# oss0430/SRFRD

Hardware: AMD Instinct MI355X
Metric: sequences/sec (higher is better)
Workload: dtype f32

## Files before the change

include/srfrd_hip.h:

```cpp
#ifndef SRFRD_HIP_H
#define SRFRD_HIP_H

#include <stddef.h>
#include <stdint.h>

#ifdef __cplusplus
extern "C" {
#endif

#define SRFRD_MAX_BLOCKS 8
#define SRFRD_MAX_D 64

enum srfrd_kind {
  SRFRD_SASREC = 0,
  SRFRD_SRFR = 1,
  SRFRD_SRFRN = 2,
  SRFRD_SRFU_B = 3,
  SRFRD_SRFU_F = 4,
  SRFRD_SRFU_R = 5
};

enum srfrd_error {
  SRFRD_E_ARG = -1,
  SRFRD_E_UNSUPPORTED = -2,
// ... 128 lines not shown
int srfrd_reduce_dense(const float* grad_slabs, int n_slabs, int64_t n_dense, float* grad_dense,
                       const float* loss_part, int B, float* stats, float* loss_out, void* stream);

int srfrd_loss_stats(const float* loss_part, int B, float* stats, float* loss_out, void* stream);

int srfrd_step_begin(uint32_t* state, double lr, double beta1, double beta2, void* stream);

int srfrd_adam_step(float* param, float* grad, float* m, float* v, int64_t n, int64_t i0, int64_t i1,
                    int64_t n_zero, double beta1, double beta2, double eps,
                    const uint32_t* state, const float* stats, uint16_t* table_bf16, int64_t n_table, void* stream);

int srfrd_adam_pack_step(const srfrd_layout* lay, float* param, float* grad, float* m, float* v, int64_t n,
                         int64_t n_table_pad, int64_t n_zero, double lr, double beta1, double beta2, double eps,
                         uint32_t* state, const float* stats, float* packed, uint16_t* table_bf16, void* stream);

int srfrd_table_to_bf16(const float* src, int64_t n, uint16_t* out, void* stream);

int srfrd_l2_norms(const float* param, const int64_t* seg_off, const int64_t* seg_len, int n_seg, int64_t n_table_pad,
                   double l2_emb, float* partial, float* l2buf, float* dense_scale, void* stream);
int srfrd_l2_apply(float* grad, const float* param, int64_t i0, int64_t i1, int64_t n_table_pad, const float* l2buf,
                   const float* dense_scale, const float* stats, void* stream);

int srfrd_loss_finalize(const float* stats, float* loss_out, void* stream);

int srfrd_user_labels(int kind, const int64_t* fake_ids, int B, int L, int64_t* labels, void* stream);

int srfrd_check_ids(const int64_t* item_a, const int64_t* item_b, const int64_t* item_c,
                    const int64_t* fake_a, const int64_t* fake_b, const int64_t* fake_c,
                    int64_t n, int64_t n_items, int64_t fake_hi, uint32_t* err_word, void* stream);

// ... 75 lines not shown
```

srfrd_amd/_lib.py:

```python
from __future__ import annotations

import ctypes as C
import os

_HERE = os.path.dirname(os.path.abspath(__file__))
LIB_PATH = os.environ.get("SRFRD_LIB_PATH") or os.path.join(_HERE, "lib", "libsrfrd_hip.so")

MAX_BLOCKS = 8
MAX_D = 64
EXCL_CAP = 4096
KINDS = {"SASRec": 0, "SRFR": 1, "SRFRN": 2, "SRFU_B": 3, "SRFU_F": 4, "SRFU_R": 5}
_ERR = {-1: "SRFRD_E_ARG (bad argument)", -2: "SRFRD_E_UNSUPPORTED (configuration outside the fused kernels: "
        "hidden width > 64, hidden width not divisible by num_heads, a debug tap of a kernel without taps, or a caller-provided "
        "scratch buffer too small for this sequence length)", -3: "SRFRD_E_DEVICE"}


class BlockOff(C.Structure):
    _fields_ = [(n, C.c_int64) for n in ("ln1_w", "ln1_b", "in_w", "in_b", "out_w", "out_b", "ln2_w", "ln2_b",
                                         "c1_w", "c1_b", "c2_w", "c2_b")]


class Layout(C.Structure):
    _fields_ = ([(n, C.c_int32) for n in ("kind", "n_items", "max_len", "d_item", "d_fake", "D", "d_out", "n_labels",
                                          "n_blocks", "n_heads", "side_rows", "side_cols", "table_bf16", "reserved0")]
# ... 25 lines not shown
    "srfrd_encoder_fwd_sched": (_i, [_LP, _P, _P, _P, _P, _P, _P, _P, _P, _P, _i, _i, _d, _u32, _P, _i64,
                                     _P, _P, _P, _P, _P, _P, _P, _P, _i64, _P, _i, _P]),
    "srfrd_encoder_bwd_sched": (_i, [_LP, _P, _P, _P, _P, _P, _P, _P, _P, _P, _i, _i, _d, _u32, _P, _i64,
                                     _P, _P, _P, _P, _P, _P, _P, _P, _P, _i, _P, _P, _P, _P, _i64, _P, _i, _P]),
    "srfrd_encoder_plan_train": (_i, [_LP, _i, _i, _i, _i, _i, _i64, _P, _i, _P]),
    "srfrd_train_scratch_floats": (_i64, [_LP, _i, _i]),
    "srfrd_encoder_train_sched": (_i, [_LP, _P, _P, _P, _P, _P, _P, _P, _P, _P, _i, _i, _d, _u32, _P, _i64,
                                       _P, _P, _P, _P, _P, _P, _P, _P, _P, _P, _i, _P, _P, _P, _P, _i64, _P, _i, _P]),
    "srfrd_table_reduce": (_i, [_P, _P, _P, _i64, _i, _P, _P]),
    "srfrd_aux_floats": (_i64, [_LP, _i, _i]),
    "srfrd_reduce_dense": (_i, [_P, _i, _i64, _P, _P, _i, _P, _P, _P]),
    "srfrd_loss_stats": (_i, [_P, _i, _P, _P, _P]),
    "srfrd_step_begin": (_i, [_P, _d, _d, _d, _P]),
    "srfrd_adam_step": (_i, [_P, _P, _P, _P, _i64, _i64, _i64, _i64, _d, _d, _d, _P, _P, _P, _i64, _P]),
    "srfrd_adam_pack_step": (_i, [_LP, _P, _P, _P, _P, _i64, _i64, _i64, _d, _d, _d, _d, _P, _P, _P, _P, _P]),
    "srfrd_table_to_bf16": (_i, [_P, _i64, _P, _P]),
    "srfrd_loss_finalize": (_i, [_P, _P, _P]),
    "srfrd_l2_norms": (_i, [_P, _P, _P, _i, _i64, _d, _P, _P, _P, _P]),
    "srfrd_l2_apply": (_i, [_P, _P, _i64, _i64, _i64, _P, _P, _P, _P]),
    "srfrd_user_labels": (_i, [_i, _P, _i, _i, _P, _P]),
    "srfrd_check_ids": (_i, [_P, _P, _P, _P, _P, _P, _i64, _i64, _i64, _P, _P]),
    "srfrd_predict_logits": (_i, [_LP, _P, _P, _P, _i, _i, _P, _i, _i64, _P, _P, _P]),
    "srfrd_topk_workspace_bytes": (_i64, [_i, _i, _i64]),
    "srfrd_logits_topk": (_i, [_LP, _P, _P, _P, _i, _i, _i64, _i64, _i, _P, _i, _P, _P, _P, _P]),
    "srfrd_topk_merge": (_i, [_P, _P, _i, _i, _i, _P, _P, _P]),
    "srfrd_excl_workspace_bytes": (_i64, [_i, _i, _i64]),
    "srfrd_logits_topk_excl": (_i, [_LP, _P, _P, _P, _i, _i, _i64, _i64, _i, _P, _i, _P, _P, _i, _P, _P, _P, _P, _P]),
    "srfrd_target_rank": (_i, [_LP, _P, _P, _P, _i, _i, _i64, _i64, _i, _P, _P, _P, _P, _i, _i, _P, _P, _P, _P]),
    "srfrd_rank_plan": (_i, [_LP, _i, _i, _i, _i64, _i64, _i, _i, _i, _i, _P, _i, _P]),
    "srfrd_eval_rank": (_i, [_P, _i, _i, _P, _P, _P]),
# ... 105 lines not shown
```

srfrd_amd/csrc/srfrd_optim.hip:

```cpp
#include "srfrd_dev.h"

namespace srfrd {

__global__ void __launch_bounds__(256) reduce_dense_kernel(const float* __restrict__ slabs, int n_slabs, int64_t n_dense,
                                                          float* __restrict__ grad_dense, const float* __restrict__ loss_part,
                                                          int B, float* __restrict__ stats, float* __restrict__ loss_out) {
  __shared__ float part[4][64];
  const int lane = threadIdx.x & 63, wave = threadIdx.x >> 6;
  const int64_t i = (int64_t)blockIdx.x * 64 + lane;
  float s0 = 0.f, s1 = 0.f, s2 = 0.f, s3 = 0.f;
  if (i < n_dense) {
    int w = wave;
    for (; w + 28 < n_slabs; w += 32) {
      const float a0 = slabs[(int64_t)w * n_dense + i], a1 = slabs[(int64_t)(w + 4) * n_dense + i];
      const float a2 = slabs[(int64_t)(w + 8) * n_dense + i], a3 = slabs[(int64_t)(w + 12) * n_dense + i];
      const float a4 = slabs[(int64_t)(w + 16) * n_dense + i], a5 = slabs[(int64_t)(w + 20) * n_dense + i];
      const float a6 = slabs[(int64_t)(w + 24) * n_dense + i], a7 = slabs[(int64_t)(w + 28) * n_dense + i];
      s0 += a0; s1 += a1; s2 += a2; s3 += a3;
      s0 += a4; s1 += a5; s2 += a6; s3 += a7;
    }
    for (; w + 12 < n_slabs; w += 16) {
      s0 += slabs[(int64_t)w * n_dense + i];
      s1 += slabs[(int64_t)(w + 4) * n_dense + i];
      s2 += slabs[(int64_t)(w + 8) * n_dense + i];
      s3 += slabs[(int64_t)(w + 12) * n_dense + i];
    }
    for (; w < n_slabs; w += 4) s0 += slabs[(int64_t)w * n_dense + i];
  }
  part[wave][lane] = (s0 + s1) + (s2 + s3);
  __syncthreads();
  if (wave == 0 && i < n_dense) grad_dense[i] = (part[0][lane] + part[1][lane]) + (part[2][lane] + part[3][lane]);
  if (blockIdx.x == 0 && loss_part != nullptr && stats != nullptr) {
    __shared__ float red[4][3];
    float a0 = 0.f, a1 = 0.f, a2 = 0.f;
    for (int b = threadIdx.x; b < B; b += blockDim.x) {
      a0 += loss_part[(int64_t)b * 3 + 0];
      a1 += loss_part[(int64_t)b * 3 + 1];
      a2 += loss_part[(int64_t)b * 3 + 2];
    }
    a0 = wave_sum(a0); a1 = wave_sum(a1); a2 = wave_sum(a2);
    if (lane == 0) { red[wave][0] = a0; red[wave][1] = a1; red[wave][2] = a2; }
    __syncthreads();
    if (threadIdx.x < 3) {
      float s = 0.f;
      for (int w = 0; w < 4; ++w) s += red[w][threadIdx.x];
      stats[threadIdx.x] = s;
      red[0][threadIdx.x] = s;
    }
    if (threadIdx.x == 3) stats[3] = 0.f;
    if (loss_out != nullptr) {
      __syncthreads();
      if (threadIdx.x == 0) loss_out[0] = red[0][0] / red[0][2] + red[0][1] / red[0][2];
    }
  }
}

__global__ void __launch_bounds__(256) loss_stats_kernel(const float* __restrict__ loss_part, int B, float* __restrict__ stats,
                                                        float* __restrict__ loss_out) {
  __shared__ float red[4][3];
  const int lane = threadIdx.x & 63, wave = threadIdx.x >> 6;
  float a0 = 0.f, a1 = 0.f, a2 = 0.f;
  for (int b = threadIdx.x; b < B; b += blockDim.x) {
    a0 += loss_part[(int64_t)b * 3 + 0];
    a1 += loss_part[(int64_t)b * 3 + 1];
    a2 += loss_part[(int64_t)b * 3 + 2];
  }
  a0 = wave_sum(a0); a1 = wave_sum(a1); a2 = wave_sum(a2);
  if (lane == 0) { red[wave][0] = a0; red[wave][1] = a1; red[wave][2] = a2; }
// ... 21 lines not shown
  for (int64_t j = i; j < n && keys[j] == key; ++j)
    if (lane < di) acc += contrib[order[j] * di + lane];
  if (lane < di) grad_table[key * di + lane] = acc;
}

__global__ void step_begin_kernel(uint32_t* state, double lr, double b1, double b2) {
  if (threadIdx.x == 0 && blockIdx.x == 0) step_advance(state, lr, b1, b2);
}

__device__ __forceinline__ void adam_one(float& p, float g, float& m, float& v, float b1, float b2, float eps,
                                         float step_size, float bc2s) {
  m = m * b1 + (1.0f - b1) * g;
  v = v * b2 + ((1.0f - b2) * g) * g;
  const float denom = sqrtf(v) / bc2s + eps;
  p = p - step_size * (m / denom);
}

__device__ __forceinline__ void shadow_store4(uint16_t* __restrict__ shadow, int64_t i, int64_t n_shadow, const float4& p4) {
  const uint16_t h0 = f32_to_bf16(p4.x), h1 = f32_to_bf16(p4.y), h2 = f32_to_bf16(p4.z), h3 = f32_to_bf16(p4.w);
  if (i + 3 < n_shadow) {
    *reinterpret_cast<uint2*>(shadow + i) = make_uint2((uint32_t)h0 | ((uint32_t)h1 << 16), (uint32_t)h2 | ((uint32_t)h3 << 16));
  } else {
    shadow[i] = h0;
    if (i + 1 < n_shadow) shadow[i + 1] = h1;
    if (i + 2 < n_shadow) shadow[i + 2] = h2;
  }
}

__global__ void __launch_bounds__(256) table_to_bf16_kernel(const float* __restrict__ src, int64_t n, uint16_t* __restrict__ out) {
  const int64_t stride = (int64_t)gridDim.x * blockDim.x;
// ... 55 lines not shown
    else if (off >= o.c2_w && off < o.c2_w + DD) { m = 5; e = off - o.c2_w; }
    else return;
    mat = b * 6 + m; N = D; K = D;
  }
  (void)N;
  const int n = e / K, k = e - n * K;
  auto slot = [](int kk, int nn) {
    const int rem = kk & 15;
    return ((nn >> 4) << 10) | ((kk >> 4) << 8) | ((((rem & 3) << 4) | (nn & 15)) << 2) | (rem >> 2);
  };
  float* base = packed + (int64_t)mat * 2 * kPackFloats;
  base[slot(k, n)] = val;
  base[kPackFloats + slot(n, k)] = val;
}

__global__ void __launch_bounds__(512) adam_pack_kernel(float* __restrict__ param, float* __restrict__ grad, float* __restrict__ m,
                                                       float* __restrict__ v, int64_t n, int64_t n_tab, int64_t n_zero, float b1,
                                                       float b2, float eps, uint32_t* __restrict__ state,
                                                       const float* __restrict__ stats, Dims dims, float* __restrict__ packed,
                                                       double lr, double b1d, double b2d, uint16_t* __restrict__ shadow,
                                                       int64_t n_shadow) {
  const float step_size = ((const float*)state)[4];
  const float bc2s = ((const float*)state)[5];
  const float gscale = stats ? 1.0f / stats[2] : 1.0f;
  const int64_t nvec = n >> 2;
  const int64_t stride = (int64_t)gridDim.x * blockDim.x;
  const int64_t w_lo = n_tab + dims.blk0;
  for (int64_t q = (int64_t)blockIdx.x * blockDim.x + threadIdx.x; q < nvec; q += stride) {
    const int64_t i = q << 2;
    float4 p4 = *reinterpret_cast<float4*>(param + i);
    float4 g4 = *reinterpret_cast<const float4*>(grad + i);
    float4 m4 = *reinterpret_cast<float4*>(m + i);
    float4 v4 = *reinterpret_cast<float4*>(v + i);
    adam_one(p4.x, g4.x * gscale, m4.x, v4.x, b1, b2, eps, step_size, bc2s);
    adam_one(p4.y, g4.y * gscale, m4.y, v4.y, b1, b2, eps, step_size, bc2s);
    adam_one(p4.z, g4.z * gscale, m4.z, v4.z, b1, b2, eps, step_size, bc2s);
    adam_one(p4.w, g4.w * gscale, m4.w, v4.w, b1, b2, eps, step_size, bc2s);
    *reinterpret_cast<float4*>(param + i) = p4;
    *reinterpret_cast<float4*>(m + i) = m4;
    *reinterpret_cast<float4*>(v + i) = v4;
    if (i + 3 < n_zero) *reinterpret_cast<float4*>(grad + i) = make_float4(0.f, 0.f, 0.f, 0.f);
    else if (i < n_zero) for (int k = 0; k < 4; ++k) if (i + k < n_zero) grad[i + k] = 0.f;
    if (shadow != nullptr && i < n_shadow) shadow_store4(shadow, i, n_shadow, p4);
    if (i + 3 >= w_lo) {
      pack_scatter(dims, i - n_tab, p4.x, packed);
      pack_scatter(dims, i + 1 - n_tab, p4.y, packed);
      pack_scatter(dims, i + 2 - n_tab, p4.z, packed);
      pack_scatter(dims, i + 3 - n_tab, p4.w, packed);
    }
  }
  for (int64_t i = (nvec << 2) + (int64_t)blockIdx.x * blockDim.x + threadIdx.x; i < n; i += stride) {
    float p = param[i], mm = m[i], vv = v[i];
    adam_one(p, grad[i] * gscale, mm, vv, b1, b2, eps, step_size, bc2s);
    param[i] = p; m[i] = mm; v[i] = vv;
    if (i < n_zero) grad[i] = 0.f;
    if (shadow != nullptr && i < n_shadow) shadow[i] = f32_to_bf16(p);
    if (i >= w_lo) pack_scatter(dims, i - n_tab, p, packed);
  }
  __syncthreads();
  if (threadIdx.x == 0) {
    const unsigned shard = blockIdx.x & 15u, n_shards = gridDim.x < 16u ? gridDim.x : 16u;
    const unsigned in_shard = (gridDim.x - shard + 15u) >> 4;
    if (atomicAdd(&state[8 + shard], 1u) == in_shard - 1u) {
      state[8 + shard] = 0;
      if (atomicAdd(&state[6], 1u) == n_shards - 1u) {
        state[6] = 0;
        step_advance(state, lr, b1d, b2d);
      }
    }
  }
}

__global__ void __launch_bounds__(256) l2_partial_kernel(const float* __restrict__ param, const int64_t* __restrict__ seg_off,
                                                        const int64_t* __restrict__ seg_len, int n_tw, float* __restrict__ partial) {
  __shared__ float red[4];
  const int g = blockIdx.x;
  int64_t lo, hi;
  if (g < n_tw) {
    const int64_t n = seg_len[0], per = ((n + n_tw - 1) / n_tw + 3) & ~3ll;
    lo = seg_off[0] + g * per;
    hi = seg_off[0] + (g + 1) * per < seg_off[0] + n ? seg_off[0] + (g + 1) * per : seg_off[0] + n;
  } else {
    const int k = g - n_tw + 1;
    lo = seg_off[k];
    hi = lo + seg_len[k];
// ... 100 lines not shown

extern "C" int srfrd_adam_step(float* param, float* grad, float* m, float* v, int64_t n, int64_t i0, int64_t i1,
                               int64_t n_zero, double beta1, double beta2, double eps, const uint32_t* state,
                               const float* stats, uint16_t* table_bf16, int64_t n_table, void* stream) {
  if (!param || !grad || !m || !v || !state || n <= 0 || i0 < 0 || i1 > n || i0 > i1) return SRFRD_E_ARG;
  if (i0 == i1) return 0;
  if (i0 & 3) return SRFRD_E_ARG;
  const int64_t nvec = ((i1 - i0) >> 2) + 1;
  int64_t grid = (nvec + 255) / 256;
  if (grid > 4096) grid = 4096;
  hipLaunchKernelGGL(adam_kernel, dim3((int)grid), dim3(256), 0, (hipStream_t)stream, param, grad, m, v, i0, i1, n_zero,
                     (float)beta1, (float)beta2, (float)eps, state, stats, table_bf16, table_bf16 ? n_table : 0);
  return (int)hipGetLastError();
}

extern "C" int srfrd_adam_pack_step(const srfrd_layout* lay, float* param, float* grad, float* m, float* v, int64_t n,
                                    int64_t n_table_pad, int64_t n_zero, double lr, double beta1, double beta2, double eps,
                                    uint32_t* state, const float* stats, float* packed, uint16_t* table_bf16, void* stream) {
  if (!lay || !param || !grad || !m || !v || !state || !packed || n <= 0 || n_table_pad < 0 || (n_table_pad & 3) ||
      n_table_pad + lay->n_dense > n)
    return SRFRD_E_ARG;
  if (lay->D > SRFRD_MAX_D) return SRFRD_E_UNSUPPORTED;
  Dims d = {};
  d.kind = lay->kind; d.d_item = lay->d_item; d.d_fake = lay->d_fake; d.D = lay->D; d.d_out = lay->d_out;
  d.n_labels = lay->n_labels; d.n_blocks = lay->n_blocks;
  d.off_pos = (int)lay->off_pos; d.off_side = (int)lay->off_side;
  d.blk0 = lay->n_blocks > 0 ? (int)lay->blk[0].ln1_w : 0;
  d.blk_stride = blk_stride_of(lay->D);
  d.off_lc_w = (int)lay->off_lc_w; d.off_lc_b = (int)lay->off_lc_b; d.off_ll_w = (int)lay->off_ll_w; d.off_ll_b = (int)lay->off_ll_b;
  d.n_dense = (int)lay->n_dense;
  int64_t grid = ((n >> 2) + 1 + 511) / 512;
  if (grid > 768) grid = 768;
  hipLaunchKernelGGL(adam_pack_kernel, dim3((int)grid), dim3(512), 0, (hipStream_t)stream, param, grad, m, v, n, n_table_pad,
                     n_zero, (float)beta1, (float)beta2, (float)eps, state, stats, d, packed, lr, beta1, beta2, table_bf16,
                     table_bf16 ? lay->n_table : 0);
  return (int)hipGetLastError();
}

extern "C" int srfrd_l2_norms(const float* param, const int64_t* seg_off, const int64_t* seg_len, int n_seg, int64_t n_table_pad,
                              double l2_emb, float* partial, float* l2buf, float* dense_scale, void* stream) {
  if (!param || !seg_off || !seg_len || !partial || !l2buf || !dense_scale || n_seg < 1 || n_seg > 128 || n_table_pad < 0)
    return SRFRD_E_ARG;
  const int n_tw = 240;
  hipLaunchKernelGGL(l2_partial_kernel, dim3(n_tw + n_seg - 1), dim3(256), 0, (hipStream_t)stream, param, seg_off, seg_len, n_tw,
                     partial);
  hipLaunchKernelGGL(l2_finish_kernel, dim3(1), dim3(256), 0, (hipStream_t)stream, partial, seg_off, seg_len, n_seg, n_tw,
                     n_table_pad, (float)l2_emb, l2buf, dense_scale);
  return (int)hipGetLastError();
}

// ... 17 lines not shown
```

srfrd_amd/trainer.py:

```python
from __future__ import annotations

import ctypes as C
import os

import torch
import torch.distributed as dist

import numpy as np

from . import _lib, loss_heads
from ._lib import check, ptr
from .exchange import GradExchange, exchange_active, shard_bounds
from .sampler import alias_table, negative_q

LOSSES = ("bce", "sampled_softmax", "softmax")


def flat_allreduce(flat: torch.Tensor, group=None):
    if dist.is_available() and dist.is_initialized() and dist.get_world_size(group) > 1:
        dist.all_reduce(flat, op=dist.ReduceOp.SUM, group=group)
    return flat


def _loss_config(model, loss, num_negatives, neg_counts, neg_alpha, process_group):
# ... 168 lines not shown

    def _dense_ptr(self, base):
        return C.c_void_p(base.data_ptr() + 4 * self.n_tab)

    def _ids_of(self, slot):
        ids = self.ids_ring[slot]
        fk = ids[1] if self.lay.kind != 0 else None
        pfk, nfk = (ids[3], ids[5]) if self.lay.kind == 2 else (None, None)
        p = self.model.dropout_rate if self.model.training else 0.0
        return ids, fk, pfk, nfk, p, C.c_void_p(self.state.data_ptr() + 8), self.rank * self.B

    def _enqueue_l2_apply(self, grad_ptr, param, i0, i1):
        check(_lib.lib().srfrd_l2_apply(grad_ptr, ptr(param), i0, min(i1, self.n_flat), self.n_tab, ptr(self.l2buf),
                                        ptr(self.l2_dense), ptr(self.stats), self._stream()), "srfrd_l2_apply")

    def _enqueue_fwd(self, slot: int = 0, train: bool = False):
        L_, lay, st = _lib.lib(), self.lay, self._stream()
        if self.l2 != 0.0:
            check(L_.srfrd_l2_norms(ptr(self.flat), ptr(self.seg_off), ptr(self.seg_len), self.seg_off.numel(), self.n_tab,
                                    self.l2, ptr(self.l2_partial), ptr(self.l2buf), ptr(self.l2_dense), st), "srfrd_l2_norms")
        ids, fk, pfk, nfk, p, seed_dev, seq0 = self._ids_of(slot)
        lay_t, tab = self.model._table_args()
        if self.sched_mode:
            check(L_.srfrd_seq_order(ptr(ids[0]), self.B, self.L, self.pair_stride, ptr(self.sched), st), "srfrd_seq_order")
        if train:
            check(L_.srfrd_encoder_train_sched(C.byref(lay_t), tab, self._dense_ptr(self.flat), ptr(self.packed), ptr(ids[0]), ptr(fk),
                                               ptr(ids[2]), ptr(pfk), ptr(ids[4]), ptr(nfk), self.B, self.L, p, 0, seed_dev, seq0,
                                               ptr(self.hidden), ptr(self.pl), ptr(self.nl), ptr(self.save_x), ptr(self.save_h1),
                                               ptr(self.save_aux), ptr(self.loss_part), None, None, None, 1, ptr(self.grad),
                                               ptr(self.contrib), ptr(self.slabs), ptr(self.scratch), self.n_scratch, ptr(self.sched),
                                               self.sched_mode, st), "srfrd_encoder_train_sched")
            self._enqueue_grad_tail(slot)
            return
        check(L_.srfrd_encoder_fwd_sched(C.byref(lay_t), tab, self._dense_ptr(self.flat), ptr(self.packed), ptr(ids[0]), ptr(fk), ptr(ids[2]),
                                         ptr(pfk), ptr(ids[4]), ptr(nfk), self.B, self.L, p, 0, seed_dev, seq0, ptr(self.hidden),
                                         ptr(self.pl), ptr(self.nl), ptr(self.save_x), ptr(self.save_h1), ptr(self.save_aux), ptr(self.loss_part),
                                         ptr(self.scratch), self.n_scratch, ptr(self.sched), self.sched_mode, st), "srfrd_encoder_fwd_sched")
        if self.mode == "sharded":
            check(L_.srfrd_loss_stats(ptr(self.loss_part), self.B, ptr(self.stats), None, st), "srfrd_loss_stats")

    def _enqueue_bwd(self, slot: int = 0):
        L_, lay, st = _lib.lib(), self.lay, self._stream()
        ids, fk, pfk, nfk, p, seed_dev, seq0 = self._ids_of(slot)
        lay_t, tab = self.model._table_args()
        check(L_.srfrd_encoder_bwd_sched(C.byref(lay_t), tab, self._dense_ptr(self.flat), ptr(self.packed), ptr(ids[0]), ptr(fk), ptr(ids[2]),
                                         ptr(pfk), ptr(ids[4]), ptr(nfk), self.B, self.L, p, 0, seed_dev, seq0, ptr(self.hidden),
                                         ptr(self.pl), ptr(self.nl), ptr(self.save_x), ptr(self.save_h1), ptr(self.save_aux), None, None, None, 1,
                                         ptr(self.grad), ptr(self.contrib), ptr(self.slabs), ptr(self.scratch), self.n_scratch,
                                         ptr(self.sched), self.sched_mode, st), "srfrd_encoder_bwd_sched")
        self._enqueue_grad_tail(slot)

    def _enqueue_grad_tail(self, slot: int = 0):
        L_, lay, st = _lib.lib(), self.lay, self._stream()
        ids = self.ids_ring[slot]
        if self.contrib is not None:
            torch.stack((ids[2], ids[4], ids[0]), out=self.keys)
            skeys, order = torch.sort(self.keys.view(-1), stable=True)
            check(L_.srfrd_table_reduce(ptr(skeys), ptr(order), ptr(self.contrib), skeys.numel(), lay.d_item, ptr(self.grad), st),
                  "srfrd_table_reduce")
        fuse_stats = self.mode != "sharded"
        check(L_.srfrd_reduce_dense(ptr(self.slabs), self.n_slabs, lay.n_dense, self._dense_ptr(self.grad),
                                    ptr(self.loss_part) if fuse_stats else None, self.B, ptr(self.stats) if fuse_stats else None,
                                    ptr(self.loss) if self.mode == "single" else None, st), "srfrd_reduce_dense")

    def _enqueue_ce_compute(self, slot: int = 0):
        L_, lay, st = _lib.lib(), self.lay, self._stream()
        B, L, T, di = self.B, self.L, self.B * self.L, lay.d_item
        if self.l2 != 0.0:
            check(L_.srfrd_l2_norms(ptr(self.flat), ptr(self.seg_off), ptr(self.seg_len), self.seg_off.numel(), self.n_tab,
                                    self.l2, ptr(self.l2_partial), ptr(self.l2buf), ptr(self.l2_dense), st), "srfrd_l2_norms")
        ids, fk, pfk, nfk, p, seed_dev, seq0 = self._ids_of(slot)
        lay_t, tab = self.model._table_args()
        if self.sched_mode:
            check(L_.srfrd_seq_order(ptr(ids[0]), B, L, self.pair_stride, ptr(self.sched), st), "srfrd_seq_order")
# ... 39 lines not shown
              "srfrd_reduce_dense")

    def _enqueue_compute(self, slot: int = 0):
        self._enqueue_fwd(slot)
        self._enqueue_bwd(slot)

    def _enqueue_step_compute(self, slot: int = 0):
        if self.loss_kind != "bce":
            self._enqueue_ce_compute(slot)
        elif self.mode == "single" and self.train_launch and _lib.encoder_plan_train(
                self.lay, self.B, self.L, self._train_mode, _lib.env_switches())[0]:
            self._enqueue_fwd(slot, train=True)
        else:
            self._enqueue_compute(slot)

    def _enqueue_update(self):
        L_, st = _lib.lib(), self._stream()
        if self.l2 != 0.0:
            self._enqueue_l2_apply(ptr(self.grad), self.flat, 0, self.n_flat)
        check(L_.srfrd_adam_pack_step(C.byref(self.lay), ptr(self.flat), ptr(self.grad), ptr(self.m), ptr(self.v),
                                      self.n_flat, self.n_tab, self.n_tab, self.lr, self.betas[0], self.betas[1], self.eps,
                                      ptr(self.state), ptr(self.stats), ptr(self.packed), ptr(self.model._table16), st),
              "srfrd_adam_pack_step")
        if self.mode != "single" or self.loss_kind != "bce":
            check(L_.srfrd_loss_finalize(ptr(self.stats), ptr(self.loss), st), "srfrd_loss_finalize")
        if self.l2 != 0.0:
            self.loss.add_(self.l2buf[1:2])

    def _enqueue_shard_update(self):
        L_, st, ex = _lib.lib(), self._stream(), self.ex
# ... 48 lines not shown
                h.wait()
            self._enqueue_shard_update()
            self._gather_params()
            self._enqueue_shard_finish()

    def _capture(self):
        torch.cuda.synchronize()
        keep = [self.flat, self.m, self.v, self.state, self.grad, self.stats] + ([self.shadow_pad] if self.shadow_gather else [])
        snap = [t.clone() for t in keep]
        s = torch.cuda.Stream()
        s.wait_stream(torch.cuda.current_stream())
        with torch.cuda.stream(s):
            if self.mode != "single" and self.ex.native:
                self._enqueue_dp_step()
            else:
                self._enqueue_step_compute()
                if self.mode == "sharded":
                    self._enqueue_shard_update()
                    self._enqueue_shard_finish()
                else:
                    self._enqueue_update()
        torch.cuda.current_stream().wait_stream(s)
        torch.cuda.synchronize()

        def restore():
            for dst, src in zip(keep, snap):
                dst.copy_(src)
            self.model.pack_weights()
            if not self.shadow_gather:
                self.model.refresh_bf16_table()

        restore()

        def graph_of(fn):
            g = torch.cuda.CUDAGraph()
            with torch.cuda.graph(g, capture_error_mode="thread_local"):
# ... 1 lines not shown
            return g

        self.graph_form = "one" if self.mode == "single" else "split"
        if self.mode != "single" and self.ex.native and os.environ.get("SRFRD_DP_SPLIT_GRAPHS", "") != "1":
            try:
                self._graph_one = [graph_of(lambda k=k: self._enqueue_dp_step(k)) for k in range(self.slots)]
                self.graph_form = "one"
            except Exception as e:
                self._graph_one = None
                self.graph_capture_error = repr(e)
                torch.cuda.synchronize()
                restore()
        if self.graph_form == "one" and self.mode != "single":
            pass
        elif self.mode == "single":
            self._graph_a = [graph_of(lambda k=k: (self._enqueue_step_compute(k), self._enqueue_update())) for k in range(self.slots)]
        elif self.mode == "allreduce":
            self._graph_a = [graph_of(lambda k=k: self._enqueue_compute(k)) for k in range(self.slots)]
            self._graph_b = graph_of(self._enqueue_update)
        else:
            self._graph_f = [graph_of(lambda k=k: self._enqueue_fwd(k)) for k in range(self.slots)]
            self._graph_a = [graph_of(lambda k=k: self._enqueue_bwd(k)) for k in range(self.slots)]
            self._graph_u = graph_of(self._enqueue_shard_update)
            self._graph_b = graph_of(self._enqueue_shard_finish)
        if self._graph_one is None:
            for gs in (self._graph_f, self._graph_a, [self._graph_u], [self._graph_b]):
                for g in (gs or []):
                    if g is not None:
                        g.replay()
        else:
            for g in self._graph_one:
# ... 136 lines not shown
        return self._run()

    def step_slot(self, slot: int) -> torch.Tensor:
        if not 0 <= slot < self.slots:
            raise IndexError(f"slot {slot} outside the ring of {self.slots}")
        return self._run(slot)

    def _run(self, slot: int = 0):
        if not self._fresh:
            self.refresh()
        g = self.use_graph
        if g and self._graph_a is None and self._graph_one is None:
            self._capture()
        if not g:
            if self.mode == "single":
                self._enqueue_step_compute(slot)
                self._enqueue_update()
            else:
                self._enqueue_dp_step(slot)
        elif self._graph_one is not None:
            self._graph_one[slot].replay()
        elif self.mode == "single":
            self._graph_a[slot].replay()
        elif self.mode == "allreduce":
            self._graph_a[slot].replay()
            self.ex.all_reduce(self.grad)
            self._graph_b.replay()
        else:
            self._graph_f[slot].replay()
            h = self.ex.all_reduce_stats(self.stats)
            self._graph_a[slot].replay()
            self.ex.reduce_scatter(self.grad, self.recv)
# ... 8 lines not shown
```

Baseline: 3.050 million.

## Fuse dense slab reduction, loss stats and Adam pack step into one kernel

```diff
diff --git a/include/srfrd_hip.h b/include/srfrd_hip.h
--- a/include/srfrd_hip.h
+++ b/include/srfrd_hip.h
@@ -166,6 +166,11 @@
                          int64_t n_table_pad, int64_t n_zero, double lr, double beta1, double beta2, double eps,
                          uint32_t* state, const float* stats, float* packed, uint16_t* table_bf16, void* stream);
 
+int srfrd_reduce_adam_pack_step(const srfrd_layout* lay, const float* grad_slabs, int n_slabs, const float* loss_part, int B,
+                                int L, float* stats, float* loss_out, float* param, float* grad, float* m, float* v, int64_t n,
+                                int64_t n_table_pad, int64_t n_zero, double lr, double beta1, double beta2, double eps,
+                                uint32_t* state, float* packed, uint16_t* table_bf16, void* stream);
+
 int srfrd_table_to_bf16(const float* src, int64_t n, uint16_t* out, void* stream);
 
 int srfrd_l2_norms(const float* param, const int64_t* seg_off, const int64_t* seg_len, int n_seg, int64_t n_table_pad,
diff --git a/srfrd_amd/_lib.py b/srfrd_amd/_lib.py
--- a/srfrd_amd/_lib.py
+++ b/srfrd_amd/_lib.py
@@ -63,6 +63,8 @@
     "srfrd_step_begin": (_i, [_P, _d, _d, _d, _P]),
     "srfrd_adam_step": (_i, [_P, _P, _P, _P, _i64, _i64, _i64, _i64, _d, _d, _d, _P, _P, _P, _i64, _P]),
     "srfrd_adam_pack_step": (_i, [_LP, _P, _P, _P, _P, _i64, _i64, _i64, _d, _d, _d, _d, _P, _P, _P, _P, _P]),
+    "srfrd_reduce_adam_pack_step": (_i, [_LP, _P, _i, _P, _i, _i, _P, _P, _P, _P, _P, _P, _i64, _i64, _i64, _d, _d, _d, _d,
+                                         _P, _P, _P, _P]),
     "srfrd_table_to_bf16": (_i, [_P, _i64, _P, _P]),
     "srfrd_loss_finalize": (_i, [_P, _P, _P]),
     "srfrd_l2_norms": (_i, [_P, _P, _P, _i, _i64, _d, _P, _P, _P, _P]),
diff --git a/srfrd_amd/csrc/srfrd_optim.hip b/srfrd_amd/csrc/srfrd_optim.hip
--- a/srfrd_amd/csrc/srfrd_optim.hip
+++ b/srfrd_amd/csrc/srfrd_optim.hip
@@ -1,6 +1,65 @@
 #include "srfrd_dev.h"
 
 namespace srfrd {
+
+template <bool DEEP = false>
+__device__ __forceinline__ float slab_quarter_sum(const float* __restrict__ slabs, int n_slabs, int64_t n_dense, int64_t i, int w) {
+  float s0 = 0.f, s1 = 0.f, s2 = 0.f, s3 = 0.f;
+  if constexpr (DEEP) {
+    for (; w + 60 < n_slabs; w += 64) {
+      float a[16];
+#pragma unroll
+      for (int k = 0; k < 16; ++k) a[k] = slabs[(int64_t)(w + 4 * k) * n_dense + i];
+      s0 += a[0]; s1 += a[1]; s2 += a[2]; s3 += a[3];
+      s0 += a[4]; s1 += a[5]; s2 += a[6]; s3 += a[7];
+      s0 += a[8]; s1 += a[9]; s2 += a[10]; s3 += a[11];
+      s0 += a[12]; s1 += a[13]; s2 += a[14]; s3 += a[15];
+    }
+  }
+  for (; w + 28 < n_slabs; w += 32) {
+    const float a0 = slabs[(int64_t)w * n_dense + i], a1 = slabs[(int64_t)(w + 4) * n_dense + i];
+    const float a2 = slabs[(int64_t)(w + 8) * n_dense + i], a3 = slabs[(int64_t)(w + 12) * n_dense + i];
+    const float a4 = slabs[(int64_t)(w + 16) * n_dense + i], a5 = slabs[(int64_t)(w + 20) * n_dense + i];
+    const float a6 = slabs[(int64_t)(w + 24) * n_dense + i], a7 = slabs[(int64_t)(w + 28) * n_dense + i];
+    s0 += a0; s1 += a1; s2 += a2; s3 += a3;
+    s0 += a4; s1 += a5; s2 += a6; s3 += a7;
+  }
+  for (; w + 12 < n_slabs; w += 16) {
+    s0 += slabs[(int64_t)w * n_dense + i];
+    s1 += slabs[(int64_t)(w + 4) * n_dense + i];
+    s2 += slabs[(int64_t)(w + 8) * n_dense + i];
+    s3 += slabs[(int64_t)(w + 12) * n_dense + i];
+  }
+  for (; w < n_slabs; w += 4) s0 += slabs[(int64_t)w * n_dense + i];
+  return (s0 + s1) + (s2 + s3);
+}
+
+__device__ __forceinline__ void loss_tree(const float* __restrict__ loss_part, int B, float* __restrict__ stats,
+                                          float* __restrict__ loss_out, float (*red)[3]) {
+  const int lane = threadIdx.x & 63, wave = threadIdx.x >> 6;
+  float a0 = 0.f, a1 = 0.f, a2 = 0.f;
+  if (threadIdx.x < 256) {
+    for (int b = threadIdx.x; b < B; b += 256) {
+      a0 += loss_part[(int64_t)b * 3 + 0];
+      a1 += loss_part[(int64_t)b * 3 + 1];
+      a2 += loss_part[(int64_t)b * 3 + 2];
+    }
+  }
+  a0 = wave_sum(a0); a1 = wave_sum(a1); a2 = wave_sum(a2);
+  if (lane == 0 && wave < 4) { red[wave][0] = a0; red[wave][1] = a1; red[wave][2] = a2; }
+  __syncthreads();
+  if (threadIdx.x < 3) {
+    float s = 0.f;
+    for (int w = 0; w < 4; ++w) s += red[w][threadIdx.x];
+    stats[threadIdx.x] = s;
+    red[0][threadIdx.x] = s;
+  }
+  if (threadIdx.x == 3) stats[3] = 0.f;
+  if (loss_out != nullptr) {
+    __syncthreads();
+    if (threadIdx.x == 0) loss_out[0] = red[0][0] / red[0][2] + red[0][1] / red[0][2];
+  }
+}
 
 __global__ void __launch_bounds__(256) reduce_dense_kernel(const float* __restrict__ slabs, int n_slabs, int64_t n_dense,
                                                           float* __restrict__ grad_dense, const float* __restrict__ loss_part,
@@ -8,50 +67,12 @@
   __shared__ float part[4][64];
   const int lane = threadIdx.x & 63, wave = threadIdx.x >> 6;
   const int64_t i = (int64_t)blockIdx.x * 64 + lane;
-  float s0 = 0.f, s1 = 0.f, s2 = 0.f, s3 = 0.f;
-  if (i < n_dense) {
-    int w = wave;
-    for (; w + 28 < n_slabs; w += 32) {
-      const float a0 = slabs[(int64_t)w * n_dense + i], a1 = slabs[(int64_t)(w + 4) * n_dense + i];
-      const float a2 = slabs[(int64_t)(w + 8) * n_dense + i], a3 = slabs[(int64_t)(w + 12) * n_dense + i];
-      const float a4 = slabs[(int64_t)(w + 16) * n_dense + i], a5 = slabs[(int64_t)(w + 20) * n_dense + i];
-      const float a6 = slabs[(int64_t)(w + 24) * n_dense + i], a7 = slabs[(int64_t)(w + 28) * n_dense + i];
-      s0 += a0; s1 += a1; s2 += a2; s3 += a3;
-      s0 += a4; s1 += a5; s2 += a6; s3 += a7;
-    }
-    for (; w + 12 < n_slabs; w += 16) {
-      s0 += slabs[(int64_t)w * n_dense + i];
-      s1 += slabs[(int64_t)(w + 4) * n_dense + i];
-      s2 += slabs[(int64_t)(w + 8) * n_dense + i];
-      s3 += slabs[(int64_t)(w + 12) * n_dense + i];
-    }
-    for (; w < n_slabs; w += 4) s0 += slabs[(int64_t)w * n_dense + i];
-  }
-  part[wave][lane] = (s0 + s1) + (s2 + s3);
+  part[wave][lane] = i < n_dense ? slab_quarter_sum(slabs, n_slabs, n_dense, i, wave) : 0.f;
   __syncthreads();
   if (wave == 0 && i < n_dense) grad_dense[i] = (part[0][lane] + part[1][lane]) + (part[2][lane] + part[3][lane]);
   if (blockIdx.x == 0 && loss_part != nullptr && stats != nullptr) {
     __shared__ float red[4][3];
-    float a0 = 0.f, a1 = 0.f, a2 = 0.f;
-    for (int b = threadIdx.x; b < B; b += blockDim.x) {
-      a0 += loss_part[(int64_t)b * 3 + 0];
-      a1 += loss_part[(int64_t)b * 3 + 1];
-      a2 += loss_part[(int64_t)b * 3 + 2];
-    }
-    a0 = wave_sum(a0); a1 = wave_sum(a1); a2 = wave_sum(a2);
-    if (lane == 0) { red[wave][0] = a0; red[wave][1] = a1; red[wave][2] = a2; }
-    __syncthreads();
-    if (threadIdx.x < 3) {
-      float s = 0.f;
-      for (int w = 0; w < 4; ++w) s += red[w][threadIdx.x];
-      stats[threadIdx.x] = s;
-      red[0][threadIdx.x] = s;
-    }
-    if (threadIdx.x == 3) stats[3] = 0.f;
-    if (loss_out != nullptr) {
-      __syncthreads();
-      if (threadIdx.x == 0) loss_out[0] = red[0][0] / red[0][2] + red[0][1] / red[0][2];
-    }
+    loss_tree(loss_part, B, stats, loss_out, red);
   }
 }
 
@@ -103,6 +124,14 @@
   v = v * b2 + ((1.0f - b2) * g) * g;
   const float denom = sqrtf(v) / bc2s + eps;
   p = p - step_size * (m / denom);
+}
+
+__device__ __forceinline__ void adam_one_pinned(float& p, float g, float& m, float& v, float b1, float b2, float eps,
+                                                float step_size, float bc2s) {
+  m = __fmaf_rn(1.0f - b1, g, __fmul_rn(m, b1));
+  v = __fmaf_rn(g, __fmul_rn(1.0f - b2, g), __fmul_rn(v, b2));
+  const float denom = __fadd_rn(sqrtf(v) / bc2s, eps);
+  p = __fmaf_rn(-step_size, m / denom, p);
 }
 
 __device__ __forceinline__ void shadow_store4(uint16_t* __restrict__ shadow, int64_t i, int64_t n_shadow, const float4& p4) {
@@ -188,6 +217,56 @@
   base[kPackFloats + slot(n, k)] = val;
 }
 
+template <bool PIN>
+__device__ __forceinline__ float4 adam_vec4_step(float* __restrict__ param, float* __restrict__ grad, float* __restrict__ m,
+                                                 float* __restrict__ v, int64_t i, int64_t n_zero, float b1, float b2, float eps,
+                                                 float step_size, float bc2s, float gscale, uint16_t* __restrict__ shadow,
+                                                 int64_t n_shadow, float4 p4, float4 g4, float4 m4, float4 v4) {
+  if constexpr (PIN) {
+    adam_one_pinned(p4.x, g4.x * gscale, m4.x, v4.x, b1, b2, eps, step_size, bc2s);
+    adam_one_pinned(p4.y, g4.y * gscale, m4.y, v4.y, b1, b2, eps, step_size, bc2s);
+    adam_one_pinned(p4.z, g4.z * gscale, m4.z, v4.z, b1, b2, eps, step_size, bc2s);
+    adam_one_pinned(p4.w, g4.w * gscale, m4.w, v4.w, b1, b2, eps, step_size, bc2s);
+  } else {
+    adam_one(p4.x, g4.x * gscale, m4.x, v4.x, b1, b2, eps, step_size, bc2s);
+    adam_one(p4.y, g4.y * gscale, m4.y, v4.y, b1, b2, eps, step_size, bc2s);
+    adam_one(p4.z, g4.z * gscale, m4.z, v4.z, b1, b2, eps, step_size, bc2s);
+    adam_one(p4.w, g4.w * gscale, m4.w, v4.w, b1, b2, eps, step_size, bc2s);
+  }
+  *reinterpret_cast<float4*>(param + i) = p4;
+  *reinterpret_cast<float4*>(m + i) = m4;
+  *reinterpret_cast<float4*>(v + i) = v4;
+  if (i + 3 < n_zero) *reinterpret_cast<float4*>(grad + i) = make_float4(0.f, 0.f, 0.f, 0.f);
+  else if (i < n_zero) for (int k = 0; k < 4; ++k) if (i + k < n_zero) grad[i + k] = 0.f;
+  if (shadow != nullptr && i < n_shadow) shadow_store4(shadow, i, n_shadow, p4);
+  return p4;
+}
+template <bool PIN>
+__device__ __forceinline__ float4 adam_vec4(float* __restrict__ param, float* __restrict__ grad, float* __restrict__ m,
+                                            float* __restrict__ v, int64_t i, int64_t n_zero, float b1, float b2, float eps,
+                                            float step_size, float bc2s, float gscale, uint16_t* __restrict__ shadow, int64_t n_shadow) {
+  const float4 p4 = *reinterpret_cast<float4*>(param + i);
+  const float4 g4 = *reinterpret_cast<const float4*>(grad + i);
+  const float4 m4 = *reinterpret_cast<float4*>(m + i);
+  const float4 v4 = *reinterpret_cast<float4*>(v + i);
+  return adam_vec4_step<PIN>(param, grad, m, v, i, n_zero, b1, b2, eps, step_size, bc2s, gscale, shadow, n_shadow, p4, g4, m4, v4);
+}
+
+__device__ __forceinline__ void step_ticket(uint32_t* __restrict__ state, double lr, double b1d, double b2d) {
+  __syncthreads();
+  if (threadIdx.x == 0) {
+    const unsigned shard = blockIdx.x & 15u, n_shards = gridDim.x < 16u ? gridDim.x : 16u;
+    const unsigned in_shard = (gridDim.x - shard + 15u) >> 4;
+    if (atomicAdd(&state[8 + shard], 1u) == in_shard - 1u) {
+      state[8 + shard] = 0;
+      if (atomicAdd(&state[6], 1u) == n_shards - 1u) {
+        state[6] = 0;
+        step_advance(state, lr, b1d, b2d);
+      }
+    }
+  }
+}
+
 __global__ void __launch_bounds__(512) adam_pack_kernel(float* __restrict__ param, float* __restrict__ grad, float* __restrict__ m,
                                                        float* __restrict__ v, int64_t n, int64_t n_tab, int64_t n_zero, float b1,
                                                        float b2, float eps, uint32_t* __restrict__ state,
@@ -202,20 +281,7 @@
   const int64_t w_lo = n_tab + dims.blk0;
   for (int64_t q = (int64_t)blockIdx.x * blockDim.x + threadIdx.x; q < nvec; q += stride) {
     const int64_t i = q << 2;
-    float4 p4 = *reinterpret_cast<float4*>(param + i);
-    float4 g4 = *reinterpret_cast<const float4*>(grad + i);
-    float4 m4 = *reinterpret_cast<float4*>(m + i);
-    float4 v4 = *reinterpret_cast<float4*>(v + i);
-    adam_one(p4.x, g4.x * gscale, m4.x, v4.x, b1, b2, eps, step_size, bc2s);
-    adam_one(p4.y, g4.y * gscale, m4.y, v4.y, b1, b2, eps, step_size, bc2s);
-    adam_one(p4.z, g4.z * gscale, m4.z, v4.z, b1, b2, eps, step_size, bc2s);
-    adam_one(p4.w, g4.w * gscale, m4.w, v4.w, b1, b2, eps, step_size, bc2s);
-    *reinterpret_cast<float4*>(param + i) = p4;
-    *reinterpret_cast<float4*>(m + i) = m4;
-    *reinterpret_cast<float4*>(v + i) = v4;
-    if (i + 3 < n_zero) *reinterpret_cast<float4*>(grad + i) = make_float4(0.f, 0.f, 0.f, 0.f);
-    else if (i < n_zero) for (int k = 0; k < 4; ++k) if (i + k < n_zero) grad[i + k] = 0.f;
-    if (shadow != nullptr && i < n_shadow) shadow_store4(shadow, i, n_shadow, p4);
+    const float4 p4 = adam_vec4<false>(param, grad, m, v, i, n_zero, b1, b2, eps, step_size, bc2s, gscale, shadow, n_shadow);
     if (i + 3 >= w_lo) {
       pack_scatter(dims, i - n_tab, p4.x, packed);
       pack_scatter(dims, i + 1 - n_tab, p4.y, packed);
@@ -231,18 +297,98 @@
     if (shadow != nullptr && i < n_shadow) shadow[i] = f32_to_bf16(p);
     if (i >= w_lo) pack_scatter(dims, i - n_tab, p, packed);
   }
-  __syncthreads();
-  if (threadIdx.x == 0) {
-    const unsigned shard = blockIdx.x & 15u, n_shards = gridDim.x < 16u ? gridDim.x : 16u;
-    const unsigned in_shard = (gridDim.x - shard + 15u) >> 4;
-    if (atomicAdd(&state[8 + shard], 1u) == in_shard - 1u) {
-      state[8 + shard] = 0;
-      if (atomicAdd(&state[6], 1u) == n_shards - 1u) {
-        state[6] = 0;
-        step_advance(state, lr, b1d, b2d);
+  step_ticket(state, lr, b1d, b2d);
+}
+
+__global__ void __launch_bounds__(512) reduce_adam_pack_kernel(const float* __restrict__ slabs, int n_slabs, int64_t n_dense,
+                                                              const float* __restrict__ loss_part, int B, float* __restrict__ stats,
+                                                              float* __restrict__ loss_out, float* __restrict__ param,
+                                                              float* __restrict__ grad, float* __restrict__ m, float* __restrict__ v,
+                                                              int64_t n, int64_t n_tab, int64_t n_zero, float b1, float b2, float eps,
+                                                              uint32_t* __restrict__ state, Dims dims, float* __restrict__ packed,
+                                                              double lr, double b1d, double b2d, uint16_t* __restrict__ shadow,
+                                                              int64_t n_shadow, int dense_first, int n_dense_blocks) {
+  __shared__ float part[2][4][64];
+  __shared__ float red[4][3];
+  __shared__ float cred[8];
+  const int tid = threadIdx.x, lane = tid & 63, wave = tid >> 6;
+  const float step_size = ((const float*)state)[4];
+  const float bc2s = ((const float*)state)[5];
+  const int bid = blockIdx.x;
+  const bool dense_role = bid >= dense_first && bid < dense_first + n_dense_blocks;
+  const bool table_role = !dense_role || gridDim.x == 1;
+  float cnt = 0.f;
+  for (int b = tid; b < B; b += 512) cnt += loss_part[(int64_t)b * 3 + 2];
+  if (bid == 0) loss_tree(loss_part, B, stats, loss_out, red);
+  const int half = wave >> 2, w4 = wave & 3;
+  const int64_t n_pairs = (((n_dense + 63) >> 6) + 1) >> 1;
+  const int64_t u0 = bid - dense_first;
+  float mine = 0.f, p0 = 0.f, m0 = 0.f, v0 = 0.f;
+  if (dense_role && u0 < n_pairs) {
+    const int64_t j = ((u0 << 1) + half) * 64 + lane;
+    if (j < n_dense) {
+      if (w4 == 0) { p0 = param[n_tab + j]; m0 = m[n_tab + j]; v0 = v[n_tab + j]; }
+      mine = slab_quarter_sum<true>(slabs, n_slabs, n_dense, j, w4);
+    }
+  }
+  const int64_t nvec = n_tab >> 2;
+  const int64_t t_blocks = (int64_t)gridDim.x - (gridDim.x == 1 ? 0 : n_dense_blocks);
+  const int64_t t_index = bid == 0 ? 0 : bid - n_dense_blocks;
+  const int64_t stride = t_blocks * 512;
+  int64_t q = t_index * 512 + tid;
+  float4 p4, g4, m4, v4;
+  const bool first = table_role && bid != 0 && q < nvec;
+  if (first) {
+    p4 = *reinterpret_cast<const float4*>(param + (q << 2));
+    g4 = *reinterpret_cast<const float4*>(grad + (q << 2));
+    m4 = *reinterpret_cast<const float4*>(m + (q << 2));
+    v4 = *reinterpret_cast<const float4*>(v + (q << 2));
+  }
+  cnt = wave_sum(cnt);
+  if (lane == 0) cred[wave] = cnt;
+  part[half][w4][lane] = mine;
+  __syncthreads();
+  float count = 0.f;
+  for (int w = 0; w < 8; ++w) count += cred[w];
+  const float gscale = 1.0f / count;
+  const int64_t w_lo = n_tab + dims.blk0;
+  if (dense_role) {
+    for (int64_t u = u0; u < n_pairs; u += n_dense_blocks) {
+      const int64_t j = ((u << 1) + half) * 64 + lane;
+      if (u != u0) {
+        part[half][w4][lane] = j < n_dense ? slab_quarter_sum<true>(slabs, n_slabs, n_dense, j, w4) : 0.f;
+        __syncthreads();
       }
-    }
-  }
+      if (w4 == 0 && j < n_dense) {
+        const float gd = (part[half][0][lane] + part[half][1][lane]) + (part[half][2][lane] + part[half][3][lane]);
+        const int64_t i = n_tab + j;
+        grad[i] = gd;
+        float p = p0, mm = m0, vv = v0;
+        if (u != u0) { p = param[i]; mm = m[i]; vv = v[i]; }
+        adam_one_pinned(p, gd * gscale, mm, vv, b1, b2, eps, step_size, bc2s);
+        param[i] = p; m[i] = mm; v[i] = vv;
+        if (i >= w_lo) pack_scatter(dims, j, p, packed);
+      }
+      __syncthreads();
+    }
+  }
+  if (bid == 0) {
+    for (int64_t i = n_tab + n_dense + tid; i < n; i += 512) {
+      float p = param[i], mm = m[i], vv = v[i];
+      adam_one_pinned(p, grad[i] * gscale, mm, vv, b1, b2, eps, step_size, bc2s);
+      param[i] = p; m[i] = mm; v[i] = vv;
+      if (i >= w_lo) pack_scatter(dims, i - n_tab, p, packed);
+    }
+  }
+  if (table_role) {
+    if (first) {
+      adam_vec4_step<true>(param, grad, m, v, q << 2, n_zero, b1, b2, eps, step_size, bc2s, gscale, shadow, n_shadow, p4, g4, m4, v4);
+      q += stride;
+    }
+    for (; q < nvec; q += stride)
+      adam_vec4<true>(param, grad, m, v, q << 2, n_zero, b1, b2, eps, step_size, bc2s, gscale, shadow, n_shadow);
+  }
+  step_ticket(state, lr, b1d, b2d);
 }
 
 __global__ void __launch_bounds__(256) l2_partial_kernel(const float* __restrict__ param, const int64_t* __restrict__ seg_off,
@@ -373,13 +519,7 @@
   return (int)hipGetLastError();
 }
 
-extern "C" int srfrd_adam_pack_step(const srfrd_layout* lay, float* param, float* grad, float* m, float* v, int64_t n,
-                                    int64_t n_table_pad, int64_t n_zero, double lr, double beta1, double beta2, double eps,
-                                    uint32_t* state, const float* stats, float* packed, uint16_t* table_bf16, void* stream) {
-  if (!lay || !param || !grad || !m || !v || !state || !packed || n <= 0 || n_table_pad < 0 || (n_table_pad & 3) ||
-      n_table_pad + lay->n_dense > n)
-    return SRFRD_E_ARG;
-  if (lay->D > SRFRD_MAX_D) return SRFRD_E_UNSUPPORTED;
+static Dims optim_dims(const srfrd_layout* lay) {
   Dims d = {};
   d.kind = lay->kind; d.d_item = lay->d_item; d.d_fake = lay->d_fake; d.D = lay->D; d.d_out = lay->d_out;
   d.n_labels = lay->n_labels; d.n_blocks = lay->n_blocks;
@@ -388,11 +528,49 @@
   d.blk_stride = blk_stride_of(lay->D);
   d.off_lc_w = (int)lay->off_lc_w; d.off_lc_b = (int)lay->off_lc_b; d.off_ll_w = (int)lay->off_ll_w; d.off_ll_b = (int)lay->off_ll_b;
   d.n_dense = (int)lay->n_dense;
+  return d;
+}
+
+extern "C" int srfrd_adam_pack_step(const srfrd_layout* lay, float* param, float* grad, float* m, float* v, int64_t n,
+                                    int64_t n_table_pad, int64_t n_zero, double lr, double beta1, double beta2, double eps,
+                                    uint32_t* state, const float* stats, float* packed, uint16_t* table_bf16, void* stream) {
+  if (!lay || !param || !grad || !m || !v || !state || !packed || n <= 0 || n_table_pad < 0 || (n_table_pad & 3) ||
+      n_table_pad + lay->n_dense > n)
+    return SRFRD_E_ARG;
+  if (lay->D > SRFRD_MAX_D) return SRFRD_E_UNSUPPORTED;
+  const Dims d = optim_dims(lay);
   int64_t grid = ((n >> 2) + 1 + 511) / 512;
   if (grid > 768) grid = 768;
   hipLaunchKernelGGL(adam_pack_kernel, dim3((int)grid), dim3(512), 0, (hipStream_t)stream, param, grad, m, v, n, n_table_pad,
                      n_zero, (float)beta1, (float)beta2, (float)eps, state, stats, d, packed, lr, beta1, beta2, table_bf16,
                      table_bf16 ? lay->n_table : 0);
+  return (int)hipGetLastError();
+}
+
+extern "C" int srfrd_reduce_adam_pack_step(const srfrd_layout* lay, const float* grad_slabs, int n_slabs, const float* loss_part,
+                                           int B, int L, float* stats, float* loss_out, float* param, float* grad, float* m,
+                                           float* v, int64_t n, int64_t n_table_pad, int64_t n_zero, double lr, double beta1,
+                                           double beta2, double eps, uint32_t* state, float* packed, uint16_t* table_bf16,
+                                           void* stream) {
+  if (!lay || !grad_slabs || !loss_part || !stats || !loss_out || !param || !grad || !m || !v || !state || !packed) return SRFRD_E_ARG;
+  if (n_slabs <= 0 || B <= 0 || L <= 0 || lay->n_dense <= 0 || n <= 0 || n_table_pad < 0 || (n_table_pad & 3) ||
+      n_table_pad + lay->n_dense > n || n_zero < 0 || n_zero > n_table_pad || lay->n_table > n_table_pad)
+    return SRFRD_E_ARG;
+  if (lay->D > SRFRD_MAX_D) return SRFRD_E_UNSUPPORTED;
+  if ((int64_t)B * L >= (1ll << 24)) return SRFRD_E_UNSUPPORTED;
+  const Dims d = optim_dims(lay);
+  int64_t grid = ((n >> 2) + 1 + 511) / 512;
+  if (grid > 768) grid = 768;
+  const int64_t n_pairs = (((lay->n_dense + 63) >> 6) + 1) >> 1;
+  const double dense_bytes = 4.0 * n_slabs * (double)lay->n_dense, table_bytes = 32.0 * (double)n_table_pad;
+  int64_t nd = (int64_t)((double)grid * dense_bytes / (dense_bytes + table_bytes) + 0.5);
+  if (nd > n_pairs) nd = n_pairs;
+  if (nd > grid - 1) nd = grid - 1;
+  if (nd < 1) nd = 1;
+  hipLaunchKernelGGL(reduce_adam_pack_kernel, dim3((int)grid), dim3(512), 0, (hipStream_t)stream, grad_slabs, n_slabs,
+                     (int64_t)lay->n_dense, loss_part, B, stats, loss_out, param, grad, m, v, n, n_table_pad, n_zero, (float)beta1,
+                     (float)beta2, (float)eps, state, d, packed, lr, beta1, beta2, table_bf16, table_bf16 ? lay->n_table : 0,
+                     grid > 1 ? 1 : 0, (int)nd);
   return (int)hipGetLastError();
 }
 
diff --git a/srfrd_amd/trainer.py b/srfrd_amd/trainer.py
--- a/srfrd_amd/trainer.py
+++ b/srfrd_amd/trainer.py
@@ -206,7 +206,7 @@
         check(_lib.lib().srfrd_l2_apply(grad_ptr, ptr(param), i0, min(i1, self.n_flat), self.n_tab, ptr(self.l2buf),
                                         ptr(self.l2_dense), ptr(self.stats), self._stream()), "srfrd_l2_apply")
 
-    def _enqueue_fwd(self, slot: int = 0, train: bool = False):
+    def _enqueue_fwd(self, slot: int = 0, train: bool = False, reduce: bool = True):
         L_, lay, st = _lib.lib(), self.lay, self._stream()
         if self.l2 != 0.0:
             check(L_.srfrd_l2_norms(ptr(self.flat), ptr(self.seg_off), ptr(self.seg_len), self.seg_off.numel(), self.n_tab,
@@ -222,7 +222,10 @@
                                                ptr(self.save_aux), ptr(self.loss_part), None, None, None, 1, ptr(self.grad),
                                                ptr(self.contrib), ptr(self.slabs), ptr(self.scratch), self.n_scratch, ptr(self.sched),
                                                self.sched_mode, st), "srfrd_encoder_train_sched")
-            self._enqueue_grad_tail(slot)
+            if reduce:
+                self._enqueue_grad_tail(slot)
+            else:
+                self._enqueue_table_reduce(slot)
             return
         check(L_.srfrd_encoder_fwd_sched(C.byref(lay_t), tab, self._dense_ptr(self.flat), ptr(self.packed), ptr(ids[0]), ptr(fk), ptr(ids[2]),
                                          ptr(pfk), ptr(ids[4]), ptr(nfk), self.B, self.L, p, 0, seed_dev, seq0, ptr(self.hidden),
@@ -242,7 +245,7 @@
                                          ptr(self.sched), self.sched_mode, st), "srfrd_encoder_bwd_sched")
         self._enqueue_grad_tail(slot)
 
-    def _enqueue_grad_tail(self, slot: int = 0):
+    def _enqueue_table_reduce(self, slot: int = 0):
         L_, lay, st = _lib.lib(), self.lay, self._stream()
         ids = self.ids_ring[slot]
         if self.contrib is not None:
@@ -250,6 +253,10 @@
             skeys, order = torch.sort(self.keys.view(-1), stable=True)
             check(L_.srfrd_table_reduce(ptr(skeys), ptr(order), ptr(self.contrib), skeys.numel(), lay.d_item, ptr(self.grad), st),
                   "srfrd_table_reduce")
+
+    def _enqueue_grad_tail(self, slot: int = 0):
+        L_, lay, st = _lib.lib(), self.lay, self._stream()
+        self._enqueue_table_reduce(slot)
         fuse_stats = self.mode != "sharded"
         check(L_.srfrd_reduce_dense(ptr(self.slabs), self.n_slabs, lay.n_dense, self._dense_ptr(self.grad),
                                     ptr(self.loss_part) if fuse_stats else None, self.B, ptr(self.stats) if fuse_stats else None,
@@ -319,6 +326,23 @@
         else:
             self._enqueue_compute(slot)
 
+    def _fused_tail(self):
+        return (self.loss_kind == "bce" and self.mode == "single" and self.train_launch and self.l2 == 0.0
+                and bool(_lib.encoder_plan_train(self.lay, self.B, self.L, self._train_mode, _lib.env_switches())[0]))
+
+    def _enqueue_step(self, slot: int = 0):
+        if self._fused_tail():
+            self._enqueue_fwd(slot, train=True, reduce=False)
+            L_, st = _lib.lib(), self._stream()
+            check(L_.srfrd_reduce_adam_pack_step(C.byref(self.lay), ptr(self.slabs), self.n_slabs, ptr(self.loss_part), self.B, self.L,
+                                                 ptr(self.stats), ptr(self.loss), ptr(self.flat), ptr(self.grad), ptr(self.m),
+                                                 ptr(self.v), self.n_flat, self.n_tab, self.n_tab, self.lr, self.betas[0],
+                                                 self.betas[1], self.eps, ptr(self.state), ptr(self.packed),
+                                                 ptr(self.model._table16), st), "srfrd_reduce_adam_pack_step")
+        else:
+            self._enqueue_step_compute(slot)
+            self._enqueue_update()
+
     def _enqueue_update(self):
         L_, st = _lib.lib(), self._stream()
         if self.l2 != 0.0:
@@ -397,12 +421,15 @@
             if self.mode != "single" and self.ex.native:
                 self._enqueue_dp_step()
             else:
-                self._enqueue_step_compute()
-                if self.mode == "sharded":
-                    self._enqueue_shard_update()
-                    self._enqueue_shard_finish()
+                if self.mode == "single":
+                    self._enqueue_step()
                 else:
-                    self._enqueue_update()
+                    self._enqueue_step_compute()
+                    if self.mode == "sharded":
+                        self._enqueue_shard_update()
+                        self._enqueue_shard_finish()
+                    else:
+                        self._enqueue_update()
         torch.cuda.current_stream().wait_stream(s)
         torch.cuda.synchronize()
 
@@ -434,7 +461,7 @@
         if self.graph_form == "one" and self.mode != "single":
             pass
         elif self.mode == "single":
-            self._graph_a = [graph_of(lambda k=k: (self._enqueue_step_compute(k), self._enqueue_update())) for k in range(self.slots)]
+            self._graph_a = [graph_of(lambda k=k: self._enqueue_step(k)) for k in range(self.slots)]
         elif self.mode == "allreduce":
             self._graph_a = [graph_of(lambda k=k: self._enqueue_compute(k)) for k in range(self.slots)]
             self._graph_b = graph_of(self._enqueue_update)
@@ -601,8 +628,7 @@
             self._capture()
         if not g:
             if self.mode == "single":
-                self._enqueue_step_compute(slot)
-                self._enqueue_update()
+                self._enqueue_step(slot)
             else:
                 self._enqueue_dp_step(slot)
         elif self._graph_one is not None:
```

New measurement: 3.075 million, median of 6. About the same (+0.8%).
